# socom20/speech-cloner

Hardware: AMD Instinct MI355X
Metric: mel frames/sec (higher is better)
Workload: dtype bf16; 1 GPU; full: STFT+mel front-end on batch 32 x 4 s @ 16 kHz (configs[1] input) -> 64 windows of 400 frames -> encoder (enc_14 weights) + decoder (hp/decoder_cfg_d.json sizes, random init), 64 windows per launch, independent steps pipelined over 10 HIP streams; batch=32, samples=64000, windows=64, model_dtype=bfloat16, streams=10, parallelism=utterance-sharded x1, no collective

## Files before the change

speech-cloner_amd/csrc/vc_api.hip:

```cpp
#include <cstdarg>
#include <atomic>
#include <cstdio>
#include <cstring>
#include "vc_common.h"

namespace vc {

static thread_local char g_err[512] = "";

char* last_error_buf() { return g_err; }

int set_error(int code, const char* fmt, ...) {
    va_list ap;
    va_start(ap, fmt);
    vsnprintf(g_err, sizeof(g_err), fmt, ap);
    va_end(ap);
    return code;
}

static std::atomic<int> g_opt[OPT_COUNT];
static const struct { const char* name; Option id; } k_opts[] = {
    {"bank256", OPT_BANK256}, {"bank256_xcd", OPT_BANK256_XCD}, {"conv256", OPT_CONV256},
    {"conv256_min_k", OPT_CONV256_MINK}, {"conv256_wm", OPT_CONV256_WM}, {"proj256", OPT_PROJ256}, {"proj256_split", OPT_PROJ256_SPLIT},
    {"wgrad_xcd", OPT_WGRAD_XCD}, {"gru_mfma", OPT_GRU_MFMA}, {"fe_fused", OPT_FE_FUSED},
    {"fe_fused_spin", OPT_FE_FUSED_SPIN}, {"gru_train_resident", OPT_GRU_TRAIN_RESIDENT},
    {"prenet_lds", OPT_PRENET_LDS}, {"cbhg_front_mi", OPT_CBHG_FRONT_MI}, {"gemm16_split", OPT_GEMM16_SPLIT},
    {"f32_f16x3", OPT_F32_F16X3}, {"gru_f32_wide", OPT_GRU_F32_WIDE},
};
static struct OptInit { OptInit() { for (auto& o : g_opt) o.store(-1); } } g_opt_init;

int opt(Option o) { return g_opt[o].load(std::memory_order_relaxed); }

static __global__ void zero_words_kernel(unsigned* __restrict__ p, size_t n) {
    for (size_t i = (size_t)blockIdx.x * blockDim.x + threadIdx.x; i < n; i += (size_t)gridDim.x * blockDim.x) p[i] = 0u;
}

hipError_t zero_async(void* d_p, size_t bytes, hipStream_t st) {
    if (bytes % 4) return hipErrorInvalidValue;
    const size_t n = bytes / 4;
    if (n == 0) return hipSuccess;
    const size_t blocks = (n + 255) / 256;
    hipLaunchKernelGGL(zero_words_kernel, dim3((unsigned)(blocks < 1024 ? blocks : 1024)), dim3(256), 0, st,
                       static_cast<unsigned*>(d_p), n);
    return hipGetLastError();
}

}

extern "C" {

int vc_set_option(const char* name, int value) {
    VC_REQUIRE(name, "vc_set_option: NULL name");
    for (const auto& o : vc::k_opts)
        if (!std::strcmp(o.name, name)) {
            vc::g_opt[o.id].store(value);
            return VC_OK;
        }
    return vc::set_error(VC_ERR_INVALID, "vc_set_option: unknown option %s", name);
}

int vc_get_option(const char* name, int* value) {
    VC_REQUIRE(name && value, "vc_get_option: NULL argument");
    for (const auto& o : vc::k_opts)
        if (!std::strcmp(o.name, name)) { *value = vc::g_opt[o.id].load(); return VC_OK; }
    return vc::set_error(VC_ERR_INVALID, "vc_get_option: unknown option %s", name);
}

int vc_version(void) { return VC_ABI_VERSION; }
const char* vc_last_error(void) { return vc::last_error_buf(); }
const char* vc_target_arch(void) { return "gfx950"; }

}
```

speech-cloner_amd/csrc/vc_bank256.hip:

```cpp
#include <cstdlib>
#include "vc_device.h"
#include "vc_bank256.h"

using vc::f32x16, vc::f32x4, vc::bf16x8, vc::bf16x4, vc::u32x4;

namespace {

constexpr int NT = 512;
constexpr int BM = 256;
constexpr int A_ROWS = 288;
constexpr int A_BYTES = A_ROWS * 128;
constexpr int B_BYTES = 256 * 128;
constexpr int COEF_OFF = 2 * A_BYTES + 2 * B_BYTES;
constexpr int LDS_BYTES = COEF_OFF + 2 * 256 * 4;

__global__ void __launch_bounds__(NT, 1)
bank256_kernel(Bank256Args a) {
    extern __shared__ __attribute__((aligned(16))) char smem[];
    char* const As = smem;
    char* const Bs = smem + 2 * A_BYTES;

    const int tid = threadIdx.x, lane = tid & 63;
    const int wid = __builtin_amdgcn_readfirstlane(tid >> 6);
    const int wr = wid >> 2, wc = wid & 3;
    int psel, rt, ks = 0;
    if (a.ksplit > 1) {
        const int q = blockIdx.x >> 3;
        ks = q % a.ksplit;
        rt = (q / a.ksplit) * 8 + (blockIdx.x & 7);
        psel = 0;
        if (rt * BM >= a.M) return;
    } else if (a.xcd_tiles > 0) {
        const int xcd = blockIdx.x & 7;
        int slot = blockIdx.x >> 3;
        psel = -1; rt = 0;
#pragma unroll
        for (int sg = 0; sg < 4; ++sg) {
            const int cnt = a.seg_count[xcd][sg];
            if (psel < 0 && slot < cnt) { psel = a.seg_pair[xcd][sg]; rt = a.seg_first[xcd][sg] + slot; }
            slot -= cnt;
        }
        if (psel < 0) return;
    } else {
        psel = a.n_pairs - 1 - (int)blockIdx.y;
        rt = blockIdx.x;
    }
    const Bank256Pair pr = a.p[psel];
    const int m0 = rt * (a.pool ? BM - 1 : BM);
    const int ntap = pr.taps0 + pr.extra;
    const int nslab_all = a.Cin >> 6;
    const int cs0 = ks * nslab_all / a.ksplit;
    const int nslab = (ks + 1) * nslab_all / a.ksplit - cs0;
    const int ntiles = nslab * ntap;
    const int pad_l = pr.pad_l;
    const __bf16* X = reinterpret_cast<const __bf16*>(a.X);

    const int srow = lane >> 3;
    const int pslot = lane & 7;
    const __bf16* a_src[5];
#pragma unroll
    for (int q = 0; q < 5; ++q) {
        const int rho = (q * 8 + wid) * 8 + srow;
        const int g = min(max(m0 - pad_l + rho, 0), a.M - 1);
        const int slot = pslot ^ ((rho >> 1) & 7);
        a_src[q] = X + (size_t)g * a.ldx + slot * 8 + cs0 * 64;
    }
    const int a_rows_needed = BM + ntap - 1;
    const __bf16* b_src[4];
#pragma unroll
    for (int q = 0; q < 4; ++q) {
        const int n = (q * 8 + wid) * 8 + srow;
        const int slot = pslot ^ ((n >> 1) & 7);
        const bool left = n < 128;
        const __bf16* Bt = reinterpret_cast<const __bf16*>(left ? pr.Bt0 : pr.Bt1);
        const int K = (left ? pr.taps0 : ntap) * a.Cin;
        b_src[q] = Bt + (size_t)(n & 127) * K + slot * 8 + cs0 * 64;
    }
    auto stageA = [&](int cs, int buf) {
        char* dst = As + buf * A_BYTES + wid * 1024;
#pragma unroll
        for (int q = 0; q < 5; ++q) {
            const int rb = q * 8 + wid;
            if (rb * 8 < a_rows_needed && rb < A_ROWS / 8) vc::glds16(a_src[q] + cs * 64, dst + q * 8192);
        }
    };
    auto stageB = [&](int n, int buf) {
        const int cs = n / ntap, j = n - cs * ntap;
        const int koffR = j * a.Cin + cs * 64;
        const int koffL = min(j, pr.taps0 - 1) * a.Cin + cs * 64;
        char* dst = Bs + buf * B_BYTES + wid * 1024;
#pragma unroll
        for (int q = 0; q < 4; ++q)
            if (q >= 2 || j < pr.taps0) vc::glds16(b_src[q] + (q < 2 ? koffL : koffR), dst + q * 8192);
    };

    const int li = lane & 31, lh = lane >> 5;
    const int a_row0 = wr * 128 + li;
    const int xb = (li >> 1) & 7;
    int b_off[4];
#pragma unroll
    for (int s = 0; s < 4; ++s) b_off[s] = (wc * 64 + li) * 128 + (((2 * s + lh) ^ xb) << 4);
    int jlo[4], jhi[4];
#pragma unroll
    for (int i = 0; i < 4; ++i) vc::same_tap_range(min(m0 + wr * 128 + i * 32 + li, a.M - 1), a.T, pad_l, jlo[i], jhi[i]);
    const bool left_wave = wc < 2;
    int J_lo = max(max(jlo[0], jlo[1]), max(jlo[2], jlo[3]));
    int J_hi = min(min(jhi[0], jhi[1]), min(jhi[2], jhi[3]));
    vc::wave_tap_range(J_lo, J_hi);
    if (left_wave) J_hi = min(J_hi, pr.taps0);

    f32x16 acc[4][2];
#pragma unroll
    for (int i = 0; i < 4; ++i)
#pragma unroll
        for (int c = 0; c < 2; ++c)
#pragma unroll
            for (int r = 0; r < 16; ++r) acc[i][c][r] = 0.0f;

    bf16x8 fa[2][4], fb[2][2];
    int a_base = 0, a_o[4];
    auto tap_setup = [&](int n) {
        const int cs = n / ntap, j = n - cs * ntap;
        const int rho = a_row0 + j;
        const int x = (rho >> 1) & 7;
        a_base = (cs & 1) * A_BYTES + rho * 128;
#pragma unroll
        for (int s = 0; s < 4; ++s) a_o[s] = ((2 * s + lh) ^ x) << 4;
        return j;
    };
    auto load_frags = [&](int set, int s, int bbuf) {
        const char* ap = As + a_base + a_o[s];
#pragma unroll
        for (int i = 0; i < 4; ++i) fa[set][i] = *reinterpret_cast<const bf16x8*>(ap + i * 4096);
        const char* bp = Bs + bbuf * B_BYTES + b_off[s];
        fb[set][0] = *reinterpret_cast<const bf16x8*>(bp);
        fb[set][1] = *reinterpret_cast<const bf16x8*>(bp + 4096);
    };

    {
        float* coef = reinterpret_cast<float*>(smem + COEF_OFF);
        const int ch = tid & 255, oc = (ch < 128 ? pr.c_off0 : pr.c_off1) + (ch & 127);
        const float* src = tid < 256 ? a.epi_scale : a.epi_shift;
        coef[tid] = src ? src[oc] : (tid < 256 ? 1.0f : 0.0f);
    }
    stageA(0, 0);
    stageB(0, 0);
    asm volatile("s_waitcnt vmcnt(0)" ::: "memory");
    __syncthreads();
    if (ntiles > 1) stageB(1, 1);
    if (nslab > 1) stageA(1, 1);
    int j = tap_setup(0);
    load_frags(0, 0, 0);

#ifndef B256_RP
#define B256_RP 2
#endif
    auto tile = [&](int n, const bool need_mask) {
        const bool active = !(left_wave && j >= pr.taps0);
        if (!active) {
            asm volatile("s_waitcnt vmcnt(0) lgkmcnt(0)" ::: "memory");
            __syncthreads();
            if (n + 2 < ntiles) stageB(n + 2, n & 1);
            if (n + 1 < ntiles) {
                const int cs1 = (n + 1) / ntap;
                if ((n + 1) - cs1 * ntap == 0 && cs1 + 1 < nslab) stageA(cs1 + 1, (cs1 + 1) & 1);
                j = tap_setup(n + 1);
                load_frags(0, 0, (n + 1) & 1);
            }
            return;
        }
        bool v[4];
#pragma unroll
        for (int i = 0; i < 4; ++i) v[i] = j >= jlo[i] && j < jhi[i];
        const bf16x8 zero = {};
        int jn = j;
#pragma unroll
        for (int s = 0; s < 4; ++s) {
            const int cur = s & 1, nxt = cur ^ 1;
            bool have_next = true;
            int nb = n & 1;
            if (s == 3) {
                asm volatile("s_waitcnt vmcnt(0) lgkmcnt(0)" ::: "memory");
                __syncthreads();
                if (n + 2 < ntiles) stageB(n + 2, n & 1);
                have_next = n + 1 < ntiles;
                if (have_next) {
                    const int cs1 = (n + 1) / ntap;
                    if ((n + 1) - cs1 * ntap == 0 && cs1 + 1 < nslab) stageA(cs1 + 1, (cs1 + 1) & 1);
                    jn = tap_setup(n + 1);
                }
                nb = (n + 1) & 1;
            }
            const int sn = (s + 1) & 3;
            const char* ap = As + a_base + a_o[sn];
            const char* bp = Bs + nb * B_BYTES + b_off[sn];
            if (need_mask) {
#pragma unroll
                for (int i = 0; i < 4; ++i) fa[cur][i] = v[i] ? fa[cur][i] : zero;
            }
            bf16x8* av = fa[cur];
#if B256_RP == 0
            if (have_next) {
#pragma unroll
                for (int i = 0; i < 4; ++i) fa[nxt][i] = *reinterpret_cast<const bf16x8*>(ap + i * 4096);
                fb[nxt][0] = *reinterpret_cast<const bf16x8*>(bp);
                fb[nxt][1] = *reinterpret_cast<const bf16x8*>(bp + 4096);
            }
#endif
            __builtin_amdgcn_s_setprio(1);
            acc[0][0] = __builtin_amdgcn_mfma_f32_32x32x16_bf16(fb[cur][0], av[0], acc[0][0], 0, 0, 0);
            acc[0][1] = __builtin_amdgcn_mfma_f32_32x32x16_bf16(fb[cur][1], av[0], acc[0][1], 0, 0, 0);
#if B256_RP != 0
            if (have_next) {
                fa[nxt][0] = *reinterpret_cast<const bf16x8*>(ap);
                fa[nxt][1] = *reinterpret_cast<const bf16x8*>(ap + 4096);
            }
#endif
            acc[1][0] = __builtin_amdgcn_mfma_f32_32x32x16_bf16(fb[cur][0], av[1], acc[1][0], 0, 0, 0);
            acc[1][1] = __builtin_amdgcn_mfma_f32_32x32x16_bf16(fb[cur][1], av[1], acc[1][1], 0, 0, 0);
#if B256_RP != 0
            if (have_next) {
                fa[nxt][2] = *reinterpret_cast<const bf16x8*>(ap + 2 * 4096);
                fa[nxt][3] = *reinterpret_cast<const bf16x8*>(ap + 3 * 4096);
            }
#endif
            acc[2][0] = __builtin_amdgcn_mfma_f32_32x32x16_bf16(fb[cur][0], av[2], acc[2][0], 0, 0, 0);
            acc[2][1] = __builtin_amdgcn_mfma_f32_32x32x16_bf16(fb[cur][1], av[2], acc[2][1], 0, 0, 0);
#if B256_RP != 0
            if (have_next) {
                fb[nxt][0] = *reinterpret_cast<const bf16x8*>(bp);
                fb[nxt][1] = *reinterpret_cast<const bf16x8*>(bp + 4096);
            }
#endif
            acc[3][0] = __builtin_amdgcn_mfma_f32_32x32x16_bf16(fb[cur][0], av[3], acc[3][0], 0, 0, 0);
            acc[3][1] = __builtin_amdgcn_mfma_f32_32x32x16_bf16(fb[cur][1], av[3], acc[3][1], 0, 0, 0);
#if B256_RP == 2
            __builtin_amdgcn_sched_group_barrier(0x008, 2, 0);
            __builtin_amdgcn_sched_group_barrier(0x100, 6, 0);
            __builtin_amdgcn_sched_group_barrier(0x008, 6, 0);
#elif B256_RP == 3
            __builtin_amdgcn_sched_group_barrier(0x008, 1, 0);
            __builtin_amdgcn_sched_group_barrier(0x100, 2, 0);
            __builtin_amdgcn_sched_group_barrier(0x008, 1, 0);
            __builtin_amdgcn_sched_group_barrier(0x100, 2, 0);
            __builtin_amdgcn_sched_group_barrier(0x008, 1, 0);
            __builtin_amdgcn_sched_group_barrier(0x100, 2, 0);
            __builtin_amdgcn_sched_group_barrier(0x008, 5, 0);
#elif B256_RP == 4
            __builtin_amdgcn_sched_group_barrier(0x008, 2, 0);
            __builtin_amdgcn_sched_group_barrier(0x100, 3, 0);
            __builtin_amdgcn_sched_group_barrier(0x008, 2, 0);
            __builtin_amdgcn_sched_group_barrier(0x100, 3, 0);
            __builtin_amdgcn_sched_group_barrier(0x008, 4, 0);
#elif B256_RP == 5
            __builtin_amdgcn_sched_group_barrier(0x008, 1, 0);
            __builtin_amdgcn_sched_group_barrier(0x100, 1, 0);
            __builtin_amdgcn_sched_group_barrier(0x008, 1, 0);
            __builtin_amdgcn_sched_group_barrier(0x100, 1, 0);
            __builtin_amdgcn_sched_group_barrier(0x008, 1, 0);
            __builtin_amdgcn_sched_group_barrier(0x100, 1, 0);
            __builtin_amdgcn_sched_group_barrier(0x008, 1, 0);
            __builtin_amdgcn_sched_group_barrier(0x100, 1, 0);
            __builtin_amdgcn_sched_group_barrier(0x008, 1, 0);
            __builtin_amdgcn_sched_group_barrier(0x100, 1, 0);
            __builtin_amdgcn_sched_group_barrier(0x008, 1, 0);
            __builtin_amdgcn_sched_group_barrier(0x100, 1, 0);
            __builtin_amdgcn_sched_group_barrier(0x008, 2, 0);
#endif
            __builtin_amdgcn_s_setprio(0);
        }
        j = jn;
    };
    for (int n = 0; n < ntiles; ++n) {
        tile(n, !(j >= J_lo && j < J_hi));
    }

    constexpr int EP = 528;
    __syncthreads();
    if (a.ksplit > 1) {
        typedef __attribute__((address_space(1))) unsigned gu32;
        gu32* const tk = (gu32*)(uintptr_t)(a.tick + 2 * rt);
        int* const tsh = reinterpret_cast<int*>(smem);
        if (tid == 0) tsh[0] = (int)__hip_atomic_fetch_add(tk, 1u, __ATOMIC_RELAXED, __HIP_MEMORY_SCOPE_AGENT);
        __syncthreads();
        const int ticket = __builtin_amdgcn_readfirstlane(tsh[0]);
        const int voff = (wid * 32 * 64 + lane) * 16;
        float* const slab0 = a.ws + (size_t)rt * (a.ksplit - 1) * 65536;
        if (ticket < a.ksplit - 1) {
            const uintptr_t base = (uintptr_t)(slab0 + (size_t)ticket * 65536);
            const unsigned b_lo = (unsigned)__builtin_amdgcn_readfirstlane((int)(unsigned)base);
            const unsigned b_hi = (unsigned)__builtin_amdgcn_readfirstlane((int)(unsigned)(base >> 32));
            const auto rs = __builtin_amdgcn_make_buffer_rsrc((void*)(((uintptr_t)b_hi << 32) | (uintptr_t)b_lo), 0, 262144, 0x00020000);
#pragma unroll
            for (int i = 0; i < 4; ++i)
#pragma unroll
                for (int c = 0; c < 2; ++c)
#pragma unroll
                    for (int q = 0; q < 4; ++q) {
                        const f32x4 v = {acc[i][c][4 * q], acc[i][c][4 * q + 1], acc[i][c][4 * q + 2], acc[i][c][4 * q + 3]};
                        __builtin_amdgcn_raw_buffer_store_b128(__builtin_bit_cast(u32x4, v), rs,
                                                               voff + ((i * 2 + c) * 4 + q) * 1024, 0, 16);
                    }
            asm volatile("s_waitcnt vmcnt(0)" ::: "memory");
            __syncthreads();
            if (tid == 0) __hip_atomic_fetch_add(tk + 1, 1u, __ATOMIC_RELAXED, __HIP_MEMORY_SCOPE_AGENT);
            return;
        }
        if (tid == 0) {
            for (unsigned spins = 0; spins < (1u << 21); ++spins) {
                if (__hip_atomic_load(tk + 1, __ATOMIC_RELAXED, __HIP_MEMORY_SCOPE_AGENT) >= (unsigned)(a.ksplit - 1)) break;
                __builtin_amdgcn_s_sleep(16);
            }
            __builtin_amdgcn_fence(__ATOMIC_ACQUIRE, "agent");
            asm volatile("s_waitcnt vmcnt(0)" ::: "memory");
        }
        __syncthreads();
        for (int sl = 0; sl < a.ksplit - 1; ++sl) {
            const __attribute__((address_space(1))) char* sp =
                (const __attribute__((address_space(1))) char*)(uintptr_t)(slab0 + (size_t)sl * 65536) + voff;
#pragma unroll
            for (int i = 0; i < 4; ++i)
#pragma unroll
                for (int c = 0; c < 2; ++c)
#pragma unroll
                    for (int q = 0; q < 4; ++q) {
                        const f32x4 v = *reinterpret_cast<const __attribute__((address_space(1))) f32x4*>(sp + ((i * 2 + c) * 4 + q) * 1024);
#pragma unroll
                        for (int e = 0; e < 4; ++e) acc[i][c][4 * q + e] += v[e];
                    }
        }
        __syncthreads();
    }
    {
#pragma unroll
        for (int c = 0; c < 2; ++c) {
#pragma unroll
            for (int q = 0; q < 4; ++q) {
                const int chp = wc * 64 + c * 32 + 8 * q + 4 * lh;
                const float4 sv = *reinterpret_cast<const float4*>(smem + COEF_OFF + chp * 4);
                const float4 bv = *reinterpret_cast<const float4*>(smem + COEF_OFF + 1024 + chp * 4);
                const float svv[4] = {sv.x, sv.y, sv.z, sv.w}, bvv[4] = {bv.x, bv.y, bv.z, bv.w};
#pragma unroll
                for (int i = 0; i < 4; ++i) {
                    bf16x4 o;
#pragma unroll
                    for (int e = 0; e < 4; ++e) {
                        float val = acc[i][c][4 * q + e] * svv[e] + bvv[e];
                        if (a.act == VC_ACT_RELU) val = fmaxf(val, 0.0f);
                        o[e] = (__bf16)val;
                    }
                    const int row = wr * 128 + i * 32 + li;
                    const int col = wc * 64 + c * 32 + 8 * q + 4 * lh;
                    *reinterpret_cast<bf16x4*>(smem + row * EP + col * 2) = o;
                }
            }
        }
    }
    __syncthreads();
    {
        const int l16 = tid & 15, hr = tid >> 4;
        __bf16* C = reinterpret_cast<__bf16*>(a.C);
        const int nrows = a.pool ? BM - 1 : BM;
#pragma unroll 4
        for (int pss = 0; pss < 16; ++pss) {
            const int h = pss * 32 + hr;
            const int row = h >> 1, half = h & 1;
            const int gm = m0 + row;
            const char* src = smem + row * EP + half * 256 + l16 * 16;
            bf16x8 vv = *reinterpret_cast<const bf16x8*>(src);
            if (a.pool && row < BM - 1) {
                const bf16x8 nx = *reinterpret_cast<const bf16x8*>(src + EP);
                const bf16x8 mx = vc::max_nonneg(vv, nx);
                vv = (min(gm, a.M - 1) % a.T == a.T - 1) ? vv : mx;
            }
            if (gm < a.M && row < nrows)
                __builtin_nontemporal_store(vv, reinterpret_cast<bf16x8*>(C + (size_t)gm * a.ldc + (half ? pr.c_off1 : pr.c_off0) + l16 * 8));
        }
    }
}

}

int vc_bank256_ksplit(int M, int nslab) {
    const int ntm = (M + BM - 1) / BM;
    return (2 * ntm <= 256 && nslab >= 8) ? 2 : 1;
}

static size_t tick_bytes(int ntm) { return vc::align256((size_t)ntm * 8); }

size_t vc_bank256_ws_bytes(int M, int ksplit) {
    if (ksplit <= 1) return 0;
    const int ntm = (M + BM - 1) / BM;
    return tick_bytes(ntm) + (size_t)ntm * (ksplit - 1) * 262144;
}

int vc_launch_bank256(const Bank256Args& a, hipStream_t st) {
    if (int rc = vc::allow_dynamic_lds<bank256_kernel>(LDS_BYTES)) return rc;
    const int stride = a.pool ? BM - 1 : BM;
    const int ntm = (a.M + stride - 1) / stride;
    Bank256Args b = a;
    if (a.ksplit > 1) {
        VC_REQUIRE(a.n_pairs == 1 && !a.pool && a.tick && (reinterpret_cast<uintptr_t>(a.tick) & 255) == 0,
                   "split K: one pair, no pooled output, 256-byte aligned workspace");
        b.ws = reinterpret_cast<float*>(reinterpret_cast<char*>(a.tick) + tick_bytes(ntm));
        b.xcd_tiles = 0;
        VC_HIP_CHECK(vc::zero_async(a.tick, tick_bytes(ntm), st));
        hipLaunchKernelGGL(bank256_kernel, dim3((unsigned)(8 * a.ksplit * ((ntm + 7) / 8))), dim3(NT), LDS_BYTES, st, b);
        VC_HIP_CHECK(hipGetLastError());
        return VC_OK;
    }
    const int xcd_mode = vc::opt(vc::OPT_BANK256_XCD);
    b.xcd_tiles = (a.n_pairs >= 8 && a.n_pairs <= 16 && ntm < 32000 && xcd_mode != 0) ? ntm : 0;
    if (b.xcd_tiles > 0) {
        for (int x = 0; x < 8; ++x)
            for (int sg = 0; sg < 4; ++sg) b.seg_pair[x][sg] = b.seg_first[x][sg] = b.seg_count[x][sg] = 0;
        const bool split = a.n_pairs == 16 && xcd_mode != 1;
        int max_slots = 0;
        for (int x = 0; x < 8; ++x) {
            int slots = 0;
            if (split) {
                const int s4 = x >> 1, half = x & 1;
                const int ranks[4] = {s4, 7 - s4, 8 + s4, 15 - s4};
                const int h0 = (ntm + 1) / 2;
                for (int sg = 0; sg < 4; ++sg) {
                    b.seg_pair[x][sg] = (int16_t)(a.n_pairs - 1 - ranks[sg]);
                    b.seg_first[x][sg] = (int16_t)(half ? h0 : 0);
                    b.seg_count[x][sg] = (int16_t)(half ? ntm - h0 : h0);
                    slots += b.seg_count[x][sg];
                }
            } else {
                int sg = 0;
                for (int gi = 0; gi < a.n_pairs; ++gi) {
                    const int r16 = gi & 15;
                    if ((r16 < 8 ? r16 : 15 - r16) != x) continue;
                    b.seg_pair[x][sg] = (int16_t)(a.n_pairs - 1 - gi);
                    b.seg_first[x][sg] = 0;
                    b.seg_count[x][sg] = (int16_t)ntm;
                    slots += ntm;
                    ++sg;
                }
            }
            max_slots = slots > max_slots ? slots : max_slots;
        }
        hipLaunchKernelGGL(bank256_kernel, dim3((unsigned)(8 * max_slots)), dim3(NT), LDS_BYTES, st, b);
    } else {
        hipLaunchKernelGGL(bank256_kernel, dim3(ntm, a.n_pairs), dim3(NT), LDS_BYTES, st, b);
    }
    VC_HIP_CHECK(hipGetLastError());
    return VC_OK;
}
```

speech-cloner_amd/csrc/vc_common.h:

```cpp
#pragma once
#include <hip/hip_runtime.h>
#include <cstdarg>
#include <cstdio>
#include "vc_hip.h"

namespace vc {

char* last_error_buf();
int set_error(int code, const char* fmt, ...);

#define VC_HIP_CHECK(expr)                                                                   \
    do {                                                                                     \
        hipError_t _e = (expr);                                                              \
        if (_e != hipSuccess)                                                                \
            return vc::set_error(VC_ERR_HIP, "%s failed: %s (%s:%d)", #expr,                 \
                                 hipGetErrorString(_e), __FILE__, __LINE__);                 \
    } while (0)

#define VC_REQUIRE(cond, ...)                                                                \
    do {                                                                                     \
        if (!(cond)) return vc::set_error(VC_ERR_INVALID, __VA_ARGS__);                      \
    } while (0)

constexpr int WAVE = 64;

enum Option {
    OPT_BANK256 = 0,
    OPT_BANK256_XCD,
    OPT_CONV256,
    OPT_CONV256_MINK,
    OPT_CONV256_WM,
    OPT_PROJ256,
    OPT_PROJ256_SPLIT,
    OPT_WGRAD_XCD,
    OPT_GRU_MFMA,
    OPT_FE_FUSED,
    OPT_FE_FUSED_SPIN,
    OPT_PRENET_LDS,
    OPT_GRU_TRAIN_RESIDENT,
    OPT_CBHG_FRONT_MI,
    OPT_GRU_F32_WIDE,
    OPT_F32_F16X3,
    OPT_GEMM16_SPLIT,
    OPT_COUNT
};
int opt(Option o);

hipError_t zero_async(void* d_p, size_t bytes, hipStream_t st);

#if defined(__HIPCC__)
template <int CTRL, int ROW_MASK>
__device__ __forceinline__ float dpp_move(float identity, float v) {
    return __int_as_float(__builtin_amdgcn_update_dpp(__float_as_int(identity), __float_as_int(v), CTRL, ROW_MASK, 0xF, false));
}
#define VC_WAVE_REDUCE(OP, ID)                                                                  \
    v = OP(v, dpp_move<0xB1, 0xF>(ID, v));                             \
    v = OP(v, dpp_move<0x4E, 0xF>(ID, v));                             \
    v = OP(v, dpp_move<0x141, 0xF>(ID, v));                                \
    v = OP(v, dpp_move<0x140, 0xF>(ID, v));          \
    v = OP(v, dpp_move<0x142, 0xA>(ID, v));                 \
    v = OP(v, dpp_move<0x143, 0xC>(ID, v));                 \
    return __int_as_float(__builtin_amdgcn_readlane(__float_as_int(v), 63));
__device__ __forceinline__ float vc_addf(float a, float b) { return a + b; }
__device__ __forceinline__ float wave_sum(float v) { VC_WAVE_REDUCE(vc_addf, 0.0f) }
__device__ __forceinline__ float wave_max(float v) { VC_WAVE_REDUCE(fmaxf, -3.402823466e38f) }
__device__ __forceinline__ float highway_gate(float hpre, float tpre, float x) {
    const float hv = fmaxf(hpre, 0.0f);
    const float e = __builtin_amdgcn_exp2f(tpre * -1.4426950408889634f);
    const float tv = __builtin_amdgcn_rcpf(1.0f + e);
    return fmaf(tv, hv - x, x);
}
__device__ __forceinline__ float wave_min(float v) { VC_WAVE_REDUCE(fminf, 3.402823466e38f) }
#undef VC_WAVE_REDUCE
#endif

}
```

Baseline: 14.12 million frames/s.

## Add register-ring tap reuse variant of bank256 conv kernel

Adds a templated RING variant of the bank256 convolution-bank kernel. A fragments for consecutive taps are kept in a rotating register ring, so each tap loads only one new fragment from LDS instead of reloading all of them. To make that work, rows are interleaved across waves, the LDS A/B staging is restructured, and the epilogue row mapping is permuted to match. The variant is selected by default when the bank pair has extra taps, and it adds complexity, register pressure, and risk of remapping errors.

Result: faster. 14.28 million frames/s (median of 6 runs) (+1.1%).

```diff
diff --git a/speech-cloner_amd/csrc/vc_api.hip b/speech-cloner_amd/csrc/vc_api.hip
--- a/speech-cloner_amd/csrc/vc_api.hip
+++ b/speech-cloner_amd/csrc/vc_api.hip
@@ -25,7 +25,7 @@
     {"wgrad_xcd", OPT_WGRAD_XCD}, {"gru_mfma", OPT_GRU_MFMA}, {"fe_fused", OPT_FE_FUSED},
     {"fe_fused_spin", OPT_FE_FUSED_SPIN}, {"gru_train_resident", OPT_GRU_TRAIN_RESIDENT},
     {"prenet_lds", OPT_PRENET_LDS}, {"cbhg_front_mi", OPT_CBHG_FRONT_MI}, {"gemm16_split", OPT_GEMM16_SPLIT},
-    {"f32_f16x3", OPT_F32_F16X3}, {"gru_f32_wide", OPT_GRU_F32_WIDE},
+    {"f32_f16x3", OPT_F32_F16X3}, {"gru_f32_wide", OPT_GRU_F32_WIDE}, {"bank256_ring", OPT_BANK256_RING},
 };
 static struct OptInit { OptInit() { for (auto& o : g_opt) o.store(-1); } } g_opt_init;
 
diff --git a/speech-cloner_amd/csrc/vc_bank256.hip b/speech-cloner_amd/csrc/vc_bank256.hip
--- a/speech-cloner_amd/csrc/vc_bank256.hip
+++ b/speech-cloner_amd/csrc/vc_bank256.hip
@@ -1,4 +1,5 @@
 #include <cstdlib>
+#include <type_traits>
 #include "vc_device.h"
 #include "vc_bank256.h"
 
@@ -14,6 +15,9 @@
 constexpr int COEF_OFF = 2 * A_BYTES + 2 * B_BYTES;
 constexpr int LDS_BYTES = COEF_OFF + 2 * 256 * 4;
 
+template <int JP> using tap_phase = std::integral_constant<int, JP>;
+
+template <bool RING>
 __global__ void __launch_bounds__(NT, 1)
 bank256_kernel(Bank256Args a) {
     extern __shared__ __attribute__((aligned(16))) char smem[];
@@ -55,8 +59,26 @@
     const int pad_l = pr.pad_l;
     const __bf16* X = reinterpret_cast<const __bf16*>(a.X);
 
+    f32x16 acc[4][2];
+    auto zero_acc = [&] {
+#pragma unroll
+        for (int i = 0; i < 4; ++i)
+#pragma unroll
+            for (int c = 0; c < 2; ++c)
+#pragma unroll
+                for (int r = 0; r < 16; ++r) acc[i][c][r] = 0.0f;
+    };
+    auto store_coef = [&] {
+        float* coef = reinterpret_cast<float*>(smem + COEF_OFF);
+        const int ch = tid & 255, oc = (ch < 128 ? pr.c_off0 : pr.c_off1) + (ch & 127);
+        const float* src = tid < 256 ? a.epi_scale : a.epi_shift;
+        coef[tid] = src ? src[oc] : (tid < 256 ? 1.0f : 0.0f);
+    };
     const int srow = lane >> 3;
     const int pslot = lane & 7;
+    const int li = lane & 31, lh = lane >> 5;
+    const bool left_wave = wc < 2;
+    if constexpr (!RING) {
     const __bf16* a_src[5];
 #pragma unroll
     for (int q = 0; q < 5; ++q) {
@@ -94,7 +116,6 @@
             if (q >= 2 || j < pr.taps0) vc::glds16(b_src[q] + (q < 2 ? koffL : koffR), dst + q * 8192);
     };
 
-    const int li = lane & 31, lh = lane >> 5;
     const int a_row0 = wr * 128 + li;
     const int xb = (li >> 1) & 7;
     int b_off[4];
@@ -103,20 +124,12 @@
     int jlo[4], jhi[4];
 #pragma unroll
     for (int i = 0; i < 4; ++i) vc::same_tap_range(min(m0 + wr * 128 + i * 32 + li, a.M - 1), a.T, pad_l, jlo[i], jhi[i]);
-    const bool left_wave = wc < 2;
     int J_lo = max(max(jlo[0], jlo[1]), max(jlo[2], jlo[3]));
     int J_hi = min(min(jhi[0], jhi[1]), min(jhi[2], jhi[3]));
     vc::wave_tap_range(J_lo, J_hi);
     if (left_wave) J_hi = min(J_hi, pr.taps0);
 
-    f32x16 acc[4][2];
-#pragma unroll
-    for (int i = 0; i < 4; ++i)
-#pragma unroll
-        for (int c = 0; c < 2; ++c)
-#pragma unroll
-            for (int r = 0; r < 16; ++r) acc[i][c][r] = 0.0f;
-
+    zero_acc();
     bf16x8 fa[2][4], fb[2][2];
     int a_base = 0, a_o[4];
     auto tap_setup = [&](int n) {
@@ -137,12 +150,7 @@
         fb[set][1] = *reinterpret_cast<const bf16x8*>(bp + 4096);
     };
 
-    {
-        float* coef = reinterpret_cast<float*>(smem + COEF_OFF);
-        const int ch = tid & 255, oc = (ch < 128 ? pr.c_off0 : pr.c_off1) + (ch & 127);
-        const float* src = tid < 256 ? a.epi_scale : a.epi_shift;
-        coef[tid] = src ? src[oc] : (tid < 256 ? 1.0f : 0.0f);
-    }
+    store_coef();
     stageA(0, 0);
     stageB(0, 0);
     asm volatile("s_waitcnt vmcnt(0)" ::: "memory");
@@ -273,6 +281,157 @@
     };
     for (int n = 0; n < ntiles; ++n) {
         tile(n, !(j >= J_lo && j < J_hi));
+    }
+    } else {
+    zero_acc();
+    store_coef();
+
+    auto opaque = [](int v) { asm volatile("" : "+v"(v)); return v; };
+    auto opaque_s = [](int v) { asm volatile("" : "+s"(v)); return v; };
+    const int a_rows_needed = BM + ntap - 1;
+    auto stageA = [&](int cs, int buf) {
+        char* dst = As + buf * A_BYTES + wid * 1024;
+        auto ka = (const __attribute__((address_space(4))) Bank256Args*)__builtin_amdgcn_kernarg_segment_ptr();
+        asm volatile("" : "+s"(ka));
+        const int M_ = ka->M, ldx_ = ka->ldx;
+        const int g0 = min(max(m0 - pad_l, 0), M_ - 1);
+        const char* const Xb = reinterpret_cast<const char*>(reinterpret_cast<const __bf16*>(ka->X) + (size_t)g0 * ldx_ + (cs0 + cs) * 64);
+        const int l = opaque(lane), sr = l >> 3, ps = l & 7;
+#pragma unroll
+        for (int q = 0; q < 5; ++q) {
+            const int rb = q * 8 + wid;
+            const int rho0 = 32 * (rb % 9) + rb / 9;
+            if (rb < A_ROWS / 8 && rho0 < a_rows_needed) {
+                const int g = min(max(m0 - pad_l + rho0 + 4 * sr, 0), M_ - 1);
+                const int slot = ps ^ ((sr >> 1) | ((rb & 1) << 2));
+                vc::glds16(Xb + (unsigned)((g - g0) * (ldx_ * 2) + slot * 16), dst + q * 8192);
+            }
+        }
+    };
+    auto stageB = [&](int cs, int j, int buf) {
+        const int cin = opaque_s(a.Cin);
+        const int KL = pr.taps0 * cin, KR = ntap * cin;
+        const char* const BbL = reinterpret_cast<const char*>(pr.Bt0);
+        const char* const BbR = reinterpret_cast<const char*>(pr.Bt1);
+        const int koffR = (j * cin + (cs0 + cs) * 64) * 2;
+        const int koffL = (min(j, pr.taps0 - 1) * cin + (cs0 + cs) * 64) * 2;
+        char* dst = Bs + buf * B_BYTES + wid * 1024;
+        const int l = opaque(lane), br = wid * 8 + (l >> 3);
+        const int bslot = ((l & 7) ^ ((br >> 1) & 7)) * 16;
+        if (j < pr.taps0) {
+            const unsigned o = br * (KL * 2) + bslot;
+            vc::glds16(BbL + koffL + o, dst);
+            vc::glds16(BbL + (size_t)KL * 128 + koffL + o, dst + 8192);
+        }
+        const unsigned o = br * (KR * 2) + bslot;
+        vc::glds16(BbR + koffR + o, dst + 2 * 8192);
+        vc::glds16(BbR + (size_t)KR * 128 + koffR + o, dst + 3 * 8192);
+    };
+
+    const int b_frag = (wc * 64 + li) * 128 + ((lh ^ ((li >> 1) & 7)) << 4);
+    int tp[4];
+    int J_lo = 0, J_hi = 0x7fffffff;
+#pragma unroll
+    for (int i = 0; i < 4; ++i) {
+        int lo, hi;
+        const int m = min(m0 + wr * 128 + 4 * li + i, a.M - 1);
+        vc::same_tap_range(m, a.T, pad_l, lo, hi);
+        tp[i] = m % a.T - pad_l;
+        J_lo = max(J_lo, lo);
+        J_hi = min(J_hi, hi);
+    }
+    vc::wave_tap_range(J_lo, J_hi);
+    if (left_wave) J_hi = min(J_hi, pr.taps0);
+
+    bf16x8 ring[4][4], fb[2][2];
+    auto a_frag = [&](int q, int k, int buf, int li_) {
+        const int r = li_ + k;
+        const int x = ((r >> 1) + 4 * q) & 7;
+        return buf * A_BYTES + (q * 72 + wr * 32) * 128 + r * 128 + ((lh ^ x) << 4);
+    };
+    auto lds128 = [&](const char* base, int off) { return *reinterpret_cast<const bf16x8*>(base + off); };
+    auto load_b = [&](int set, int s, int bbuf) {
+        const int o = bbuf * B_BYTES + (opaque(b_frag) ^ (s << 5));
+        fb[set][0] = lds128(Bs, o);
+        fb[set][1] = lds128(Bs, o + 4096);
+    };
+    auto load_ring_step = [&](int s, int buf) {
+        int l = li;
+        asm volatile("" : "+v"(l));
+#pragma unroll
+        for (int q = 0; q < 4; ++q) ring[s][q] = lds128(As, a_frag(q, 0, buf, l) ^ (s << 5));
+    };
+
+    stageA(0, 0);
+    stageB(0, 0, 0);
+    asm volatile("s_waitcnt vmcnt(0)" ::: "memory");
+    __syncthreads();
+    if (ntiles > 1) stageB(ntap > 1 ? 0 : 1, ntap > 1 ? 1 : 0, 1);
+    if (nslab > 1) stageA(1, 1);
+
+    auto turn = [&](int n, int cs, int j, bool last) {
+        asm volatile("s_waitcnt vmcnt(0) lgkmcnt(0)" ::: "memory");
+        __syncthreads();
+        if (n + 2 < ntiles) {
+            int cs2 = cs, j2 = j + 2;
+            if (j2 >= ntap) { j2 -= ntap; ++cs2; }
+            if (j2 >= ntap) { j2 -= ntap; ++cs2; }
+            stageB(cs2, j2, n & 1);
+        }
+        if (last && cs + 2 < nslab) stageA(cs + 2, cs & 1);
+    };
+    auto tile = [&](auto jp_, auto mask_, int n, int cs, int j) {
+        constexpr int JP = decltype(jp_)::value;
+        const bool last = j + 1 == ntap;
+        const bool idle = left_wave && j >= pr.taps0;
+        const int a_next = a_frag(JP, (j >> 2) + 1, cs & 1, li);
+        const bf16x8 zero = {};
+#pragma unroll
+        for (int s = 0; s < 4; ++s) {
+            const int cur = s & 1, nxt = cur ^ 1;
+            int nb = n & 1;
+            if (s == 3) {
+                turn(n, cs, j, last);
+                nb = (n + 1) & 1;
+            }
+            const auto products = [&](auto i0_, auto i1_) {
+                constexpr int I0 = decltype(i0_)::value, I1 = decltype(i1_)::value;
+                __builtin_amdgcn_s_setprio(1);
+#pragma unroll
+                for (int i = I0; i < I1; ++i) {
+                    bf16x8 f = ring[s][(i + JP) & 3];
+                    if constexpr (decltype(mask_)::value) f = (unsigned)(tp[i] + j) < (unsigned)a.T ? f : zero;
+                    acc[i][0] = __builtin_amdgcn_mfma_f32_32x32x16_bf16(fb[cur][0], f, acc[i][0], 0, 0, 0);
+                    acc[i][1] = __builtin_amdgcn_mfma_f32_32x32x16_bf16(fb[cur][1], f, acc[i][1], 0, 0, 0);
+                }
+                __builtin_amdgcn_s_setprio(0);
+            };
+            if (!idle) products(tap_phase<0>{}, tap_phase<1>{});
+            ring[s][JP] = lds128(As, a_next ^ (s << 5));
+            load_b(nxt, (s + 1) & 3, nb);
+            if (!idle) products(tap_phase<1>{}, tap_phase<4>{});
+        }
+        if (last && n + 1 < ntiles) {
+#pragma unroll
+            for (int s = 0; s < 4; ++s) load_ring_step(s, (cs + 1) & 1);
+        }
+    };
+    auto taps = [&](auto mask_) {
+#pragma unroll
+        for (int s = 0; s < 4; ++s) load_ring_step(s, 0);
+        load_b(0, 0, 0);
+        for (int cs = 0, n = 0; cs < nslab; ++cs) {
+            for (int j = 0; j < ntap; j += 4, n += 4) {
+                tile(tap_phase<0>{}, mask_, n, cs, j);
+                if (j + 1 < ntap) tile(tap_phase<1>{}, mask_, n + 1, cs, j + 1);
+                if (j + 2 < ntap) tile(tap_phase<2>{}, mask_, n + 2, cs, j + 2);
+                if (j + 3 < ntap) tile(tap_phase<3>{}, mask_, n + 3, cs, j + 3);
+            }
+            n -= -ntap & 3;
+        }
+    };
+    if (J_lo <= 0 && J_hi >= (left_wave ? pr.taps0 : ntap)) taps(std::false_type{});
+    else taps(std::true_type{});
     }
 
     constexpr int EP = 528;
@@ -349,7 +508,7 @@
                         if (a.act == VC_ACT_RELU) val = fmaxf(val, 0.0f);
                         o[e] = (__bf16)val;
                     }
-                    const int row = wr * 128 + i * 32 + li;
+                    const int row = RING ? i * 64 + wr * 32 + li : wr * 128 + i * 32 + li;
                     const int col = wc * 64 + c * 32 + 8 * q + 4 * lh;
                     *reinterpret_cast<bf16x4*>(smem + row * EP + col * 2) = o;
                 }
@@ -366,10 +525,11 @@
             const int h = pss * 32 + hr;
             const int row = h >> 1, half = h & 1;
             const int gm = m0 + row;
-            const char* src = smem + row * EP + half * 256 + l16 * 16;
+            const auto prow = [](int r) { return RING ? (r & 3) * 64 + (r >> 2) : r; };
+            const char* src = smem + prow(row) * EP + half * 256 + l16 * 16;
             bf16x8 vv = *reinterpret_cast<const bf16x8*>(src);
             if (a.pool && row < BM - 1) {
-                const bf16x8 nx = *reinterpret_cast<const bf16x8*>(src + EP);
+                const bf16x8 nx = *reinterpret_cast<const bf16x8*>(smem + prow(row + 1) * EP + half * 256 + l16 * 16);
                 const bf16x8 mx = vc::max_nonneg(vv, nx);
                 vv = (min(gm, a.M - 1) % a.T == a.T - 1) ? vv : mx;
             }
@@ -395,7 +555,10 @@
 }
 
 int vc_launch_bank256(const Bank256Args& a, hipStream_t st) {
-    if (int rc = vc::allow_dynamic_lds<bank256_kernel>(LDS_BYTES)) return rc;
+    if (int rc = vc::allow_dynamic_lds<bank256_kernel<false>, bank256_kernel<true>>(LDS_BYTES)) return rc;
+    const int ring_opt = vc::opt(vc::OPT_BANK256_RING);
+    const bool ring = ring_opt < 0 ? a.p[0].extra != 0 : ring_opt != 0;
+    const auto kern = ring ? bank256_kernel<true> : bank256_kernel<false>;
     const int stride = a.pool ? BM - 1 : BM;
     const int ntm = (a.M + stride - 1) / stride;
     Bank256Args b = a;
@@ -405,7 +568,7 @@
         b.ws = reinterpret_cast<float*>(reinterpret_cast<char*>(a.tick) + tick_bytes(ntm));
         b.xcd_tiles = 0;
         VC_HIP_CHECK(vc::zero_async(a.tick, tick_bytes(ntm), st));
-        hipLaunchKernelGGL(bank256_kernel, dim3((unsigned)(8 * a.ksplit * ((ntm + 7) / 8))), dim3(NT), LDS_BYTES, st, b);
+        hipLaunchKernelGGL(kern, dim3((unsigned)(8 * a.ksplit * ((ntm + 7) / 8))), dim3(NT), LDS_BYTES, st, b);
         VC_HIP_CHECK(hipGetLastError());
         return VC_OK;
     }
@@ -442,9 +605,9 @@
             }
             max_slots = slots > max_slots ? slots : max_slots;
         }
-        hipLaunchKernelGGL(bank256_kernel, dim3((unsigned)(8 * max_slots)), dim3(NT), LDS_BYTES, st, b);
+        hipLaunchKernelGGL(kern, dim3((unsigned)(8 * max_slots)), dim3(NT), LDS_BYTES, st, b);
     } else {
-        hipLaunchKernelGGL(bank256_kernel, dim3(ntm, a.n_pairs), dim3(NT), LDS_BYTES, st, b);
+        hipLaunchKernelGGL(kern, dim3(ntm, a.n_pairs), dim3(NT), LDS_BYTES, st, b);
     }
     VC_HIP_CHECK(hipGetLastError());
     return VC_OK;
diff --git a/speech-cloner_amd/csrc/vc_common.h b/speech-cloner_amd/csrc/vc_common.h
--- a/speech-cloner_amd/csrc/vc_common.h
+++ b/speech-cloner_amd/csrc/vc_common.h
@@ -42,6 +42,7 @@
     OPT_GRU_F32_WIDE,
     OPT_F32_F16X3,
     OPT_GEMM16_SPLIT,
+    OPT_BANK256_RING,
     OPT_COUNT
 };
 int opt(Option o);
```
